# sikoba/babble

Measured on AMD Instinct MI355X. Metric: ECDSA event verifies/sec, higher is better.
Workload: dtype u32; 1 GPU; C2: VerifyBatch of 1M signed Events per GPU (64 creators, 1x64-B tx, ~446-B bodies); per-key tables rebuilt every step; events_per_gpu=1000000, creators=64, parallelism=single, batches_in_flight=2

## Files before the change

### babble_amd/csrc/bv_api.cpp

```cpp
#include "bv_internal.h"
#include "hostscalar.h"
#include "hostsha.h"

#include <algorithm>
#include <atomic>
#include <chrono>
#include <condition_variable>
#include <cstdio>
#include <cstdlib>
#include <cstring>
#include <functional>
#include <map>
#include <new>
#include <thread>

#include <sched.h>
#include <sys/syscall.h>
#include <unistd.h>

namespace {

constexpr uint64_t kGTableBytes = BV_GTABLE_U32 * 4;
constexpr uint64_t kGSubBytes = BV_GSUB_U32 * 4;
constexpr uint64_t kGPrefixBytes = (uint64_t)BV_GPAIR_BLOCKS * 4096 * 32;
constexpr uint64_t kKTableBytes = BV_KTABLE_U32 * 4;
constexpr uint64_t kK12TableBytes = BV_K12TABLE_U32 * 4;
constexpr uint64_t kK12SubBytes = BV_K12SUB_U32 * 4;
constexpr uint64_t kK12PrefixBytes = (uint64_t)BV_K12NWIN * BV_K12ENT * 32;
constexpr uint64_t kKSubBytes = BV_KSUB_U32 * 4;
constexpr uint64_t kKPrefixBytes = (uint64_t)BV_KNWIN * (1u << BV_KW) * 32;
constexpr uint32_t kBasesPerKey = 32;
constexpr uint32_t kMaxTableKeys = 8192;
constexpr uint32_t kMaxK12Keys = 1024;
constexpr uint32_t kManyKeys = 1024;
constexpr uint64_t kLatTableItems = 4096;
#ifndef BV_PREP_M
#define BV_PREP_M 16
#endif
constexpr uint32_t kPrepM = BV_PREP_M;
constexpr uint32_t kRgWords = 33;
#ifndef BV_FUSED_KC
#define BV_FUSED_KC 1
#endif
constexpr bool kFusedKc = BV_FUSED_KC;
constexpr size_t kChunk = 16ull << 20;
constexpr size_t kSmallStage = 1ull << 20;
constexpr uint64_t kHostHashLen = 16 << 10;

}

hipError_t DevBuf::ensure(size_t bytes) {
  if (bytes <= cap) return hipSuccess;
  if (p) {
    hipError_t e = hipFree(p);
    if (e != hipSuccess) return e;
    p = nullptr;
    cap = 0;
  }
  size_t want = std::max(bytes, cap * 3 / 2);
  want = (want + 255) & ~(size_t)255;
  hipError_t e = hipMalloc(&p, want);
  if (e != hipSuccess) {
    p = nullptr;
    (void)hipGetLastError();
    return e;
  }
  cap = want;
  return hipSuccess;
}
void DevBuf::release() {
  if (p) (void)hipFree(p);
  p = nullptr;
  cap = 0;
}
hipError_t PinnedBuf::ensure(size_t bytes) {
  if (bytes <= cap) return hipSuccess;
  if (p) {
    hipError_t e = hipHostFree(p);
    if (e != hipSuccess) return e;
    p = nullptr;
    cap = 0;
  }
  size_t want = std::max(bytes, cap * 3 / 2);
  want = (want + 4095) & ~(size_t)4095;
  hipError_t e = hipHostMalloc(&p, want, flags);
  if (e != hipSuccess) {
    p = nullptr;
    (void)hipGetLastError();
    return e;
  }
  cap = want;
  return hipSuccess;
}
void PinnedBuf::release() {
  if (p) (void)hipHostFree(p);
  p = nullptr;
  cap = 0;
}

int bv_fail(bv_ctx *c, int code, const char *what, hipError_t e) {
  if (c) {
    char buf[256];
    if (e != hipSuccess)
      snprintf(buf, sizeof buf, "%s: %s", what, hipGetErrorString(e));
    else
      snprintf(buf, sizeof buf, "%s", what);
    c->err = buf;
  }
  return code;
}

#define HIPCHK(expr, code, what)                               \
  do {                                                         \
    hipError_t _e = (expr);                                    \
    if (_e != hipSuccess) return bv_fail(ctx, code, what, _e); \
  } while (0)

namespace {
std::mutex g_pin_mu;
std::map<uintptr_t, size_t> g_pinned;
}

// ... 351 lines not shown
                    &sl.kc_tabs,   &sl.defer};
    for (auto *b : sb) b->release();
    sl.pin_small.release();
    if (sl.done) (void)hipEventDestroy(sl.done);
  }
  bv_kc_release(ctx);
  ctx->pin_in.release();
  ctx->pin_out.release();
  ctx->small_io.release();
  ctx->pin_long.release();
  ctx->d_long.release();
  for (auto &sl : ctx->slot)
    for (auto &e : sl.ev)
      if (e) (void)hipEventDestroy(e);
  for (auto &e : ctx->chunk_ev)
    if (e) (void)hipEventDestroy(e);
  if (ctx->ev_done) (void)hipEventDestroy(ctx->ev_done);
  if (ctx->ev_host) (void)hipEventDestroy(ctx->ev_host);
  streams_release(ctx);
  delete ctx->pool;
  delete ctx;
}

extern "C" void *bv_last_stream(const bv_ctx *ctx) { return ctx ? (void *)ctx->last : nullptr; }

static float elapsed(hipEvent_t a, hipEvent_t b);

extern "C" int bv_get_timing(const bv_ctx *ctx, bv_timing *out) {
  if (!ctx || !out) return BV_E_ARGS;
  bv_ctx *c = const_cast<bv_ctx *>(ctx);
  std::lock_guard<std::mutex> lk(c->mu);
  *out = c->timing;
  return BV_OK;
}

int bv_run_keys(bv_ctx *ctx, const bv_batch *b, hipEvent_t keys_ready, hipEvent_t s_ready, bool kc, bool split_ok) {
  const uint64_t n_items = b->n_items;
  const uint32_t n_keys = b->n_keys;
  if (n_items > 0 && (!b->item_msg || !b->item_key || !b->r_be || !b->s_be))
    return bv_fail(ctx, BV_E_ARGS, "null item arrays");
  if (n_items > 0 && n_keys == 0) return bv_fail(ctx, BV_E_ARGS, "items without keys");
  if (n_keys > 0 && !b->key_off) return bv_fail(ctx, BV_E_ARGS, "null key_off");
  if (((uintptr_t)b->r_be | (uintptr_t)b->s_be) & 15)
    return bv_fail(ctx, BV_E_ARGS, "r_be/s_be must be 16-byte aligned");
  HIPCHK(ctx->S().kstatus.ensure(std::max<uint32_t>(n_keys, 1)), BV_E_OOM, "alloc kstatus");
  HIPCHK(ctx->S().kxy.ensure(std::max<uint32_t>(n_keys, 1) * 64ull), BV_E_OOM, "alloc kxy");
  HIPCHK(ctx->S().scratch.ensure(std::max<uint64_t>(n_items, 1) * 32), BV_E_OOM, "alloc scratch");
  HIPCHK(ctx->S().u12.ensure(std::max<uint64_t>(n_items, 1) * BV_U_STRIDE * 4), BV_E_OOM, "alloc u12");

  const uint64_t min_items = n_keys <= kManyKeys ? ctx->table_min_items : ctx->table_min_items_many;
  const bool table_mode = kc || (n_keys <= kMaxTableKeys && n_items >= min_items * n_keys) ||
                          (n_keys <= ctx->lat_table_keys && n_items <= kLatTableItems && n_items > 0);
  const int key_w = kc ? BV_KCW
                    : !table_mode ? 0
                    : (n_keys <= kMaxK12Keys && n_items >= ctx->k12_min_items * n_keys && !(ctx->flags & BV_F_K8))
                        ? 12
                        : 8;
  ctx->table_mode = table_mode;
  ctx->key_w = key_w;
  if (table_mode) {
    HIPCHK(ctx->S().rg.ensure(std::max<uint64_t>(n_items, 1) * kRgWords * 4), BV_E_OOM, "alloc R_G");
    if (!kc) {
      const uint64_t nk = std::max<uint32_t>(n_keys, 1);
      HIPCHK(ctx->S().bases_jac.ensure(nk * kBasesPerKey * 96ull), BV_E_OOM, "alloc bases");
      HIPCHK(ctx->S().key_sub.ensure(nk * (key_w == 12 ? kK12SubBytes : kKSubBytes)), BV_E_OOM,
             "alloc key sub-tables");
      HIPCHK(ctx->S().key_pscr.ensure(nk * (key_w == 12 ? kK12PrefixBytes : kKPrefixBytes)), BV_E_OOM,
             "alloc key prefix scratch");
      HIPCHK(ctx->S().key_table.ensure(nk * (key_w == 12 ? kK12TableBytes : kKTableBytes)), BV_E_OOM,
             "alloc key tables");
    }
  }
  hipEvent_t *ev = ctx->S().ev;
  HIPCHK(hipStreamWaitEvent(ctx->sstream, keys_ready, 0), BV_E_LAUNCH, "fork");
  HIPCHK(hipEventRecord(ev[E_START], ctx->sstream), BV_E_LAUNCH, "event");
  if (kc && ctx->S().kc_decoded)
    HIPCHK(hipStreamWaitEvent(ctx->sstream, ctx->S().ev[E_KCDEC], 0), BV_E_LAUNCH, "join");
  else
    HIPCHK(bvk::key_decode(ctx->sstream, n_keys, b->key_bytes, b->key_off, ctx->S().kstatus.as<uint8_t>(),
                           ctx->S().kxy.as<uint32_t>()),
           BV_E_LAUNCH, "k_key_decode");
  HIPCHK(hipEventRecord(ev[E_KDEC], ctx->sstream), BV_E_LAUNCH, "event");
  HIPCHK(hipStreamWaitEvent(ctx->sstream, s_ready, 0), BV_E_LAUNCH, "fork");
  const uint32_t M = (uint32_t)std::min<uint64_t>(kPrepM, std::max<uint64_t>(1, (n_items + 65535) / 65536));
  HIPCHK(bvk::sinv(ctx->sstream, n_items, M, (const uint32_t *)b->s_be, b->pre, ctx->S().scratch.as<uint32_t>()),
         BV_E_LAUNCH, "k_sinv");
  ctx->S().glv_split = split_ok && ctx->glv_in_sstream && table_mode && !(kc && kFusedKc);
  if (ctx->S().glv_split)
    HIPCHK(bvk::glv_split(ctx->sstream, n_items, (const uint32_t *)b->r_be, ctx->S().scratch.as<uint32_t>(),
                          ctx->S().u12.as<uint32_t>()),
           BV_E_LAUNCH, "k_glv_split");
  HIPCHK(hipEventRecord(ev[E_SINV], ctx->sstream), BV_E_LAUNCH, "event");
  HIPCHK(hipStreamWaitEvent(ctx->kstream, ev[E_KDEC], 0), BV_E_LAUNCH, "fork");
  if (!kc) {
    if (table_mode)
      HIPCHK(bvk::build_tables(ctx->kstream, key_w, n_keys, ctx->S().kxy.as<uint32_t>(), ctx->S().kstatus.as<uint8_t>(),
                               ctx->S().bases_jac.as<uint32_t>(), ctx->S().key_sub.as<uint32_t>(),
                               ctx->S().key_pscr.as<uint32_t>(), ctx->S().key_table.as<uint32_t>(), n_items),
             BV_E_LAUNCH, "key tables");
  }
  HIPCHK(hipEventRecord(ev[E_KEYS], ctx->kstream), BV_E_LAUNCH, "event");
  return BV_OK;
}

int bv_out_bufs(bv_ctx *ctx, const bv_batch *b, uint8_t *d_msg_hash, uint8_t *d_status, uint64_t *d_bits,
                bool hashed, bv_out *o) {
  const uint64_t n_msgs = b->n_msgs, n_items = b->n_items;
  o->dig = (uint32_t *)d_msg_hash;
  if (hashed || !o->dig || ((uintptr_t)o->dig & 15)) {
    HIPCHK(ctx->S().digests.ensure(std::max<uint64_t>(n_msgs, 1) * 32), BV_E_OOM, "alloc digests");
    o->dig = ctx->S().digests.as<uint32_t>();
  }
  o->status = d_status;
  if (!o->status) {
    HIPCHK(ctx->S().status.ensure(std::max<uint64_t>(n_items, 1)), BV_E_OOM, "alloc status");
    o->status = ctx->S().status.as<uint8_t>();
  }
  o->bits = d_bits;
  if (!o->bits) {
    HIPCHK(ctx->S().bits.ensure(std::max<uint64_t>((n_items + 63) / 64, 1) * 8), BV_E_OOM, "alloc bits");
    o->bits = ctx->S().bits.as<uint64_t>();
  }
  return BV_OK;
}

int bv_launch_items(bv_ctx *ctx, const bv_batch *b, const bv_out &o, hipStream_t st, bool kc, uint64_t lo,
                    uint64_t hi, int part) {
  const uint64_t n = b->n_items;
  const uint8_t *kst = ctx->S().kstatus.as<uint8_t>();
  const uint32_t *r32 = (const uint32_t *)b->r_be, *s32 = (const uint32_t *)b->s_be;
  uint32_t *w = ctx->S().scratch.as<uint32_t>(), *u12 = ctx->S().u12.as<uint32_t>();
  const bool fused = kc && kFusedKc;
  if (part == 1) {
    if (ctx->table_mode && !fused)
      HIPCHK(bvk::verify_g(st, n, lo, hi, b->item_key, r32, s32, b->pre, kst, b->item_msg, o.dig, w, u12,
                           ctx->g_table, ctx->S().rg.as<uint32_t>(), ctx->S().glv_split),
             BV_E_LAUNCH, "k_verify_g");
    return BV_OK;
  }
  if (fused)
    HIPCHK(bvk::verify_gq(st, n, lo, hi, b->item_key, r32, s32, b->pre, kst, b->item_msg, o.dig, w, ctx->g_table,
                          ctx->S().kc_tabs.as<uint64_t>(), o.status, o.bits),
           BV_E_LAUNCH, "k_verify_gq");
  else if (ctx->table_mode)
    HIPCHK(bvk::verify_q(st, ctx->key_w, n, lo, hi, b->item_key, r32, s32, b->pre, kst, u12,
                         ctx->S().key_table.as<uint32_t>(), kc ? ctx->S().kc_tabs.as<uint64_t>() : nullptr,
                         ctx->S().rg.as<uint32_t>(), o.status, o.bits),
           BV_E_LAUNCH, "k_verify_q");
  else
    HIPCHK(bvk::verify_generic(st, n, lo, hi, b->item_key, r32, s32, b->pre, kst, ctx->S().kxy.as<uint32_t>(),
                               b->item_msg, o.dig, w, ctx->g_table, o.status, o.bits),
           BV_E_LAUNCH, "k_verify_generic");
  return BV_OK;
}

int bv_item_pipe::key_part(hipStream_t ks, hipEvent_t ready) {
  if (!ctx->table_mode || !ctx->qfirst || b->n_items == 0) return BV_OK;
  hipEvent_t *ev = ctx->S().ev;
  HIPCHK(hipStreamWaitEvent(ks, ev[E_SINV], 0), BV_E_LAUNCH, "join");
  HIPCHK(hipStreamWaitEvent(ks, ready, 0), BV_E_LAUNCH, "join");
  HIPCHK(hipStreamWaitEvent(ks, ev[E_KEYS], 0), BV_E_LAUNCH, "join");
  if (kc && ks != ctx->stream) {
    HIPCHK(hipEventRecord(ev[E_KCTAB], ctx->stream), BV_E_LAUNCH, "event");
    HIPCHK(hipStreamWaitEvent(ks, ev[E_KCTAB], 0), BV_E_LAUNCH, "join");
  }
  HIPCHK(hipEventRecord(ev[E_SCALAR], ks), BV_E_LAUNCH, "event");
  HIPCHK(hipEventRecord(ev[E_JOINED], ks), BV_E_LAUNCH, "event");
// ... 761 lines not shown
```

### babble_amd/csrc/field.h

```cpp
#pragma once
#include <hip/hip_runtime.h>
#include <stdint.h>

#define DEV __host__ __device__ __forceinline__

struct fe {
  uint32_t v[8];
};
struct sc {
  uint32_t v[8];
};
#if defined(__HIP_DEVICE_COMPILE__)
#include "field_asm.h"
#endif

#define P0 0xFFFFFC2Fu
#define P1 0xFFFFFFFEu
#define PX 0xFFFFFFFFu

DEV uint32_t addc32(uint32_t a, uint32_t b, uint32_t &c) {
  uint32_t co;
  uint32_t r = __builtin_addc(a, b, c, &co);
  c = co;
  return r;
// ... 312 lines not shown
#pragma unroll
    for (int j = 0; j < 8; j++) {
      uint64_t x = (uint64_t)a.v[i] * b.v[j] + t[j] + c;
      t[j] = (uint32_t)x;
      c = x >> 32;
    }
    uint32_t cc = 0;
    t[8] = addc32(t[8], (uint32_t)c, cc);
    t[9] = cc;
    uint32_t m = t[0] * SC_NINV;
    c = 0;
#pragma unroll
    for (int j = 0; j < 8; j++) {
      uint64_t x = (uint64_t)m * SC_N[j] + t[j] + c;
      t[j] = (uint32_t)x;
      c = x >> 32;
    }
    cc = 0;
    t[8] = addc32(t[8], (uint32_t)c, cc);
    t[9] += cc;
#pragma unroll
    for (int j = 0; j < 9; j++) t[j] = t[j + 1];
    t[9] = 0;
  }
#pragma unroll
  for (int i = 0; i < 8; i++) r.v[i] = t[i];
  if (t[8] || sc_ge_n(r)) sc_sub_n(r);
}

DEV void sc_load_const(sc &r, const uint32_t *c) {
#pragma unroll
  for (int i = 0; i < 8; i++) r.v[i] = c[i];
}

DEV void sc_add(sc &r, const sc &a, const sc &b) {
  uint32_t c = 0;
#pragma unroll
  for (int i = 0; i < 8; i++) r.v[i] = addc32(a.v[i], b.v[i], c);
  if (c || sc_ge_n(r)) sc_sub_n(r);
}
DEV void sc_sub(sc &r, const sc &a, const sc &b) {
  uint32_t br = 0;
#pragma unroll
  for (int i = 0; i < 8; i++) r.v[i] = subb32(a.v[i], b.v[i], br);
  if (br) {
    uint32_t c = 0;
#pragma unroll
    for (int i = 0; i < 8; i++) r.v[i] = addc32(r.v[i], SC_N[i], c);
  }
}

static constexpr uint32_t FE_BETA[8] = {0x719501EEu, 0xC1396C28u, 0x12F58995u, 0x9CF04975u,
                                        0xAC3434E9u, 0x6E64479Eu, 0x657C0710u, 0x7AE96A2Bu};
static constexpr uint32_t GLV_G1[8] = {0x45DBB031u, 0xE893209Au, 0x71E8CA7Fu, 0x3DAA8A14u,
                                       0x9284EB15u, 0xE86C90E4u, 0xA7D46BCDu, 0x3086D221u};
static constexpr uint32_t GLV_G2[8] = {0x8AC47F71u, 0x1571B4AEu, 0x9DF506C6u, 0x221208ACu,
                                       0x0ABFE4C4u, 0x6F547FA9u, 0x010E8828u, 0xE4437ED6u};
static constexpr uint32_t GLV_MB1R[8] = {0x0AD9263Cu, 0xC50468D0u, 0xFAA6ED42u, 0x1B1C8205u,
                                         0x8AC47F71u, 0x1571B4AEu, 0x9DF506C6u, 0x221208ACu};
static constexpr uint32_t GLV_MB2R[8] = {0x6A144696u, 0x0CAC5E50u, 0xF3BA5939u, 0x1E8A8DC5u,
                                         0xBA244FCEu, 0x176CDF65u, 0x8E173580u, 0xC25575EBu};
static constexpr uint32_t GLV_LAMR[8] = {0xC9926C9Eu, 0xF07DEB3Du, 0x83C6944Cu, 0x2C93E7ADu,
                                         0x52697D91u, 0x73A96606u, 0x8558D639u, 0x53284017u};
static constexpr uint32_t SC_HALF_N[8] = {0x681B20A0u, 0xDFE92F46u, 0x57A4501Du, 0x5D576E73u,
                                          0xFFFFFFFFu, 0xFFFFFFFFu, 0xFFFFFFFFu, 0x7FFFFFFFu};

DEV void glv_mulshift(sc &c, const sc &k, const uint32_t *g) {
  fe a, b;
  uint32_t w[16];
#pragma unroll
  for (int i = 0; i < 8; i++) {
    a.v[i] = k.v[i];
    b.v[i] = g[i];
  }
  mul_512(w, a, b);
  uint32_t cy = w[11] >> 31;
#pragma unroll
  for (int i = 0; i < 4; i++) c.v[i] = addc32(w[12 + i], 0u, cy);
  c.v[4] = cy;
#pragma unroll
  for (int i = 5; i < 8; i++) c.v[i] = 0;
}

DEV void glv_split(uint32_t mag1[4], uint32_t mag2[4], uint32_t &signs, const sc &k) {
  sc c1, c2, t, r1, r2, mb;
  glv_mulshift(c1, k, GLV_G1);
  glv_mulshift(c2, k, GLV_G2);
  sc_load_const(mb, GLV_MB1R);
  sc_mont(c1, c1, mb);
  sc_load_const(mb, GLV_MB2R);
  sc_mont(c2, c2, mb);
  sc_add(r2, c1, c2);
  sc_load_const(mb, GLV_LAMR);
  sc_mont(t, r2, mb);
  sc_sub(r1, k, t);
  signs = 0;
  sc h;
  sc_load_const(h, SC_HALF_N);
  sc n;
  sc_load_const(n, SC_N);
  bool gt1 = false, gt2 = false;
  {
    bool decided = false;
#pragma unroll
    for (int i = 7; i >= 0; i--) {
      if (!decided && r1.v[i] != h.v[i]) {
        gt1 = r1.v[i] > h.v[i];
        decided = true;
      }
    }
    decided = false;
#pragma unroll
    for (int i = 7; i >= 0; i--) {
      if (!decided && r2.v[i] != h.v[i]) {
        gt2 = r2.v[i] > h.v[i];
        decided = true;
      }
    }
  }
  if (gt1) {
    sc z;
    sc_sub(z, n, r1);
    r1 = z;
    signs |= 1u;
  }
  if (gt2) {
    sc z;
    sc_sub(z, n, r2);
    r2 = z;
    signs |= 2u;
  }
#pragma unroll
  for (int i = 0; i < 4; i++) {
    mag1[i] = r1.v[i];
    mag2[i] = r2.v[i];
  }
}

#include "modinv.h"

DEV void fe_inv_var(fe &r, const fe &a) {
  fe t = a;
  fe_canon(t);
  modinfo30 mi;
  modinfo_p(mi);
  modinv_var(r.v, t.v, mi);
}

static constexpr uint32_t SC_R3[8] = {0xE9FF41EDu, 0x7BC0CFE0u, 0x44D4322Cu, 0x00176484u,
                                      0xF1D0B2DAu, 0xB1B31347u, 0x18EF116Du, 0x555D800Cu};

DEV void sc_inverse_var(sc &r, const sc &xR) {
  modinfo30 mi;
  modinfo_n(mi);
  sc t, r3;
  modinv_var(t.v, xR.v, mi);
  sc_load_const(r3, SC_R3);
  sc_mont(r, t, r3);
}
```

### babble_amd/csrc/kernels.hip

```cpp
#include <hip/hip_runtime.h>
#include <stdint.h>

#include <algorithm>
#include <cstdlib>

#include "evjson.h"
#include "hostscalar.h"

#include "verify_core.h"


#ifndef BV_SHA_WAVES
#define BV_SHA_WAVES 1
#endif
__global__ void __launch_bounds__(256, BV_SHA_WAVES) k_sha256(uint64_t n_msgs, const uint8_t *__restrict__ bytes,
                                                const uint64_t *__restrict__ off,
                                                uint32_t *__restrict__ digest_words, uint64_t max_len) {
  const uint64_t m = (uint64_t)blockIdx.x * blockDim.x + threadIdx.x;
  if (m < n_msgs && off[m + 1] - off[m] <= max_len) sha256_one(m, bytes, off, digest_words);
}

__global__ void __launch_bounds__(256) k_put_digests(uint64_t n, const uint64_t *__restrict__ idx,
                                                     const uint32_t *__restrict__ vals, uint32_t *__restrict__ dig) {
  const uint64_t t = (uint64_t)blockIdx.x * blockDim.x + threadIdx.x;
// ... 160 lines not shown

template <bool LAT>
__global__ void __launch_bounds__(64) k_table_bases(uint32_t n_bases, const uint32_t *__restrict__ bxy,
                                                    const uint8_t *__restrict__ bstatus,
                                                    uint32_t *__restrict__ bases_jac, int w, int nwin) {
  const uint32_t b = blockIdx.x * blockDim.x + threadIdx.x;
  if (b >= n_bases) return;
  if (bstatus && bstatus[b] != KS_OK) return;
  table_bases_one<LAT>(b, bxy, bases_jac, w, nwin);
}

__global__ void __launch_bounds__(64) k_table_bases_coop(uint32_t n_bases, const uint32_t *__restrict__ bxy,
                                                         const uint8_t *__restrict__ bstatus,
                                                         uint32_t *__restrict__ bases_jac, int w, int nwin) {
  const uint32_t b = blockIdx.x;
  if (b >= n_bases) return;
  if (bstatus && bstatus[b] != KS_OK) return;
  coop_bases_one(b, bxy, bases_jac, w, nwin);
}

template <int N>
__device__ __forceinline__ void block_inverse(fe *T, fe &v, uint32_t t) {
  static_assert((N & (N - 1)) == 0, "power of two");
  T[N - 1 + t] = v;
  __syncthreads();
#pragma unroll 1
  for (uint32_t n = N / 2; n >= 1; n >>= 1) {
    if (t < n) {
      const uint32_t p = n - 1 + t;
      fe a = T[2 * p + 1], b = T[2 * p + 2], r;
      fe_mul(r, a, b);
      T[p] = r;
    }
    __syncthreads();
  }
  if (t == 0) {
    fe x, root = T[0];
    fe_inv_var(x, root);
    T[0] = x;
  }
  __syncthreads();
#pragma unroll 1
  for (uint32_t n = 1; n < N; n <<= 1) {
    const uint32_t c = 2 * n - 1 + t;
    fe r;
    if (t < 2 * n) {
      fe a = T[(c - 1) / 2], b = T[(c & 1u) ? c + 1 : c - 1];
      fe_mul(r, a, b);
    }
    __syncthreads();
    if (t < 2 * n) T[c] = r;
    __syncthreads();
  }
  v = T[N - 1 + t];
}

template <int W, int NWIN, bool PHI, int BLOCK = 256, bool LAT = true>
__global__ void __launch_bounds__(BLOCK) k_table_fill(const uint32_t *__restrict__ bases_jac,
                                                      const uint8_t *__restrict__ bstatus,
                                                      uint32_t *__restrict__ table) {
  static_assert(((NWIN << W) % BLOCK) == 0, "blocks cover whole keys");
  constexpr uint64_t half_u32 = (uint64_t)NWIN * (1ull << W) * BV_ENTRY_U32;
  const uint32_t b = blockIdx.y;
  const uint32_t f = blockIdx.x * BLOCK + threadIdx.x;
  const uint32_t j = f >> W;
  const uint32_t d = f & ((1u << W) - 1u);
  const uint32_t t = threadIdx.x;
  if (bstatus && bstatus[b] != KS_OK) return;
  __shared__ fe sT[2 * BLOCK - 1];
  const uint32_t *bj = bases_jac + ((uint64_t)b * NWIN + j) * 24;
  fe bx, by, bz;
  fe_load(bx, bj);
  fe_load(by, bj + 8);
  fe_load(bz, bj + 16);
  gej R;
  bool inf;
  fe Z;
  table_point<LAT>(R, inf, Z, bx, by, d, W);
  if (!inf) fe_mul(Z, Z, bz);
  fe zi = Z;
  block_inverse<BLOCK>(sT, zi, t);
  uint32_t *entry = table + (uint64_t)b * (PHI ? 2 : 1) * half_u32 + (((uint64_t)j << W) + d) * BV_ENTRY_U32;
  table_store(entry, PHI ? entry + half_u32 : nullptr, d, R, inf, zi);
}

template <int W, int L, int NWIN>
__global__ void __launch_bounds__(256) k_table_pair(const uint32_t *__restrict__ sub,
                                                    const uint8_t *__restrict__ bstatus,
                                                    uint32_t *__restrict__ table, uint4 *__restrict__ pscr) {
  constexpr uint32_t ENT = 1u << (W - 1), E = ENT / 256u, NS = 1u << L;
  constexpr uint64_t half_u32 = ((uint64_t)NWIN * ENT + 1) * BV_ENTRY_U32;
  static_assert(half_u32 == BV_K12HALF_U32, "K12 geometry");
  const uint32_t b = blockIdx.y, j = blockIdx.x, t = threadIdx.x;
  if (bstatus && bstatus[b] != KS_OK) return;
  const int live_bits = 128 - W * (int)j;
  const uint32_t e_live = live_bits >= W - 1 ? E : ((1u << live_bits) + 1u + 255u) / 256u;
  __shared__ uint32_t sLo[NS * BV_ENTRY_U32], sHi[NS * BV_ENTRY_U32];
  __shared__ fe sT[511];
  const uint32_t *sk = sub + ((uint64_t)b * 2 * NWIN + 2 * j) * NS * BV_ENTRY_U32;
  for (uint32_t x = t; x < NS * BV_ENTRY_U32; x += 256) {
    sLo[x] = sk[x];
    sHi[x] = sk[NS * BV_ENTRY_U32 + x];
  }
  __syncthreads();
  uint4 *ps = pscr + ((uint64_t)b * NWIN + j) * E * 2 * 256 + t;
  fe acc;
  fe_set(acc, 1);
#pragma unroll 1
  for (uint32_t e = 0; e < e_live; e++) {
    const uint32_t d = k12_digit(256 * e + t, ENT), lo = d & (NS - 1), hi = d >> L;
    fe x1, y1, x2, y2, H;
    pair_load(sLo, sHi, lo, hi, x1, y1, x2, y2);
    pair_denominator(H, pair_kind(lo, hi), x1, x2);
    ps[(2 * e) * 256] = make_uint4(acc.v[0], acc.v[1], acc.v[2], acc.v[3]);
    ps[(2 * e + 1) * 256] = make_uint4(acc.v[4], acc.v[5], acc.v[6], acc.v[7]);
    fe_mul(acc, acc, H);
  }
  fe q = acc;
  block_inverse<256>(sT, q, t);
  uint32_t *base = table + (uint64_t)b * 2 * half_u32 + (uint64_t)j * ENT * BV_ENTRY_U32;
#pragma unroll 1
  for (int e = (int)e_live - 1; e >= 0; e--) {
    const uint32_t d = k12_digit(256 * e + t, ENT), lo = d & (NS - 1), hi = d >> L;
    const int kind = pair_kind(lo, hi);
    fe x1, y1, x2, y2, H, Hinv, pre;
    pair_load(sLo, sHi, lo, hi, x1, y1, x2, y2);
    pair_denominator(H, kind, x1, x2);
    const uint4 p0 = ps[(2 * e) * 256], p1 = ps[(2 * e + 1) * 256];
    pre.v[0] = p0.x; pre.v[1] = p0.y; pre.v[2] = p0.z; pre.v[3] = p0.w;
    pre.v[4] = p1.x; pre.v[5] = p1.y; pre.v[6] = p1.z; pre.v[7] = p1.w;
    fe_mul(Hinv, q, pre);
    fe_mul(q, q, H);
    uint32_t *entry = base + (uint64_t)d * BV_ENTRY_U32;
    pair_store(entry, entry + half_u32, kind, x1, y1, x2, y2, Hinv);
  }
}

template <int W, int L, int NWIN, int WPB>
__global__ void __launch_bounds__(256) k_table_pair_u(const uint32_t *__restrict__ sub,
                                                      const uint8_t *__restrict__ bstatus,
                                                      uint32_t *__restrict__ table, uint4 *__restrict__ pscr) {
  constexpr uint32_t NS = 1u << L, SUB_U32 = 2 * WPB * NS * BV_ENTRY_U32;
  constexpr uint64_t half_u32 = (uint64_t)NWIN * (1ull << W) * BV_ENTRY_U32;
  static_assert((1u << W) == 256 && W == 2 * L && half_u32 == BV_KHALF_U32 && NWIN % WPB == 0, "K8 geometry");
  const uint32_t b = blockIdx.y, j0 = blockIdx.x * WPB, t = threadIdx.x;
  if (bstatus && bstatus[b] != KS_OK) return;
  __shared__ uint32_t sS[SUB_U32];
  __shared__ fe sT[511];
  const uint32_t *sk = sub + ((uint64_t)b * 2 * NWIN + 2 * j0) * NS * BV_ENTRY_U32;
  for (uint32_t x = t; x < SUB_U32; x += 256) sS[x] = sk[x];
  __syncthreads();
  const uint32_t lo = t & (NS - 1), hi = t >> L;
  const int kind = pair_kind(lo, hi);
  uint4 *ps = pscr + ((uint64_t)b * NWIN + j0) * 2 * 256 + t;
  fe acc;
  fe_set(acc, 1);
#pragma unroll 1
  for (uint32_t e = 0; e < WPB; e++) {
    fe x1, y1, x2, y2, H;
    pair_load(sS + 2 * e * NS * BV_ENTRY_U32, sS + (2 * e + 1) * NS * BV_ENTRY_U32, lo, hi, x1, y1, x2, y2);
    pair_denominator(H, kind, x1, x2);
    if (WPB > 1) {
      ps[(2 * e) * 256] = make_uint4(acc.v[0], acc.v[1], acc.v[2], acc.v[3]);
      ps[(2 * e + 1) * 256] = make_uint4(acc.v[4], acc.v[5], acc.v[6], acc.v[7]);
    }
    fe_mul(acc, acc, H);
// ... 825 lines not shown
  if (n == 0) return hipSuccess;
  hipLaunchKernelGGL(k_key_decode, grid1(n, 64), dim3(64), 0, st, n, kb, ko, kst, kxy);
  return hipGetLastError();
}

static int k12_lat_mask(bool busy) {
  static const int env = [] {
    const char *s = getenv("BV_K12_LAT");
    return s ? atoi(s) : -1;
  }();
  return env >= 0 ? env : busy ? 1 : 3;
}

static const bool g_coop_bases = [] {
  const char *s = getenv("BV_COOP_BASES");
  return s == nullptr || atoi(s) != 0;
}();

static const uint32_t g_k8_direct_keys = [] {
  const char *s = getenv("BV_K8_DIRECT_KEYS");
  return s ? (uint32_t)atoi(s) : 24u;
}();

hipError_t build_tables(hipStream_t st, int kw, uint32_t n_bases, const uint32_t *bxy, const uint8_t *bstatus,
                        uint32_t *bases_jac, uint32_t *sub, uint32_t *pscr, uint32_t *table, uint64_t n_items) {
  const bool k8_direct = kw == 8 && n_bases <= g_k8_direct_keys;
  if (n_bases == 0) return hipSuccess;
  const int w = kw == 0 ? BV_GL : kw == 8 ? (k8_direct ? BV_KW : BV_KL) : BV_K12L;
  const int nwin = kw == 0 ? BV_GNSUB : kw == 8 ? (k8_direct ? BV_KNWIN : BV_KNSUB) : BV_K12NSUB;
  const int lat = kw == 12 ? k12_lat_mask(!lat_variant(n_items)) : 3;
  if (g_coop_bases)
    hipLaunchKernelGGL(k_table_bases_coop, dim3(n_bases), dim3(64), 0, st, n_bases, bxy, bstatus, bases_jac, w, nwin);
  else if (lat & 1)
    hipLaunchKernelGGL(k_table_bases<true>, grid1(n_bases, 64), dim3(64), 0, st, n_bases, bxy, bstatus, bases_jac, w,
                       nwin);
  else
    hipLaunchKernelGGL(k_table_bases<false>, grid1(n_bases, 64), dim3(64), 0, st, n_bases, bxy, bstatus, bases_jac, w,
                       nwin);
  hipError_t e = hipGetLastError();
  if (e != hipSuccess) return e;
  if (kw == 0) {
    hipLaunchKernelGGL((k_table_fill<BV_GL, BV_GNSUB, false>), dim3(BV_GNSUB * ((1u << BV_GL) / 256u), 1), dim3(256),
                       0, st, bases_jac, bstatus, sub);
    e = hipGetLastError();
    if (e != hipSuccess) return e;
    for (uint32_t j = 0; j < BV_GNWIN; j++) {
      const int live_bits = 256 - BV_GW * (int)j;
      const uint64_t live = live_bits >= BV_GW - 1 ? BV_GENT : (1ull << live_bits) + 1;
      const uint32_t blocks = (uint32_t)((live + 4095) / 4096);
      for (uint32_t c0 = 0; c0 < blocks; c0 += BV_GPAIR_BLOCKS) {
        const uint32_t nb = blocks - c0 < BV_GPAIR_BLOCKS ? blocks - c0 : BV_GPAIR_BLOCKS;
        hipLaunchKernelGGL((k_table_pair_g<BV_GW, BV_GL>), dim3(nb), dim3(256), 0, st, sub, table, (uint4 *)pscr, j,
                           c0);
        e = hipGetLastError();
        if (e != hipSuccess) return e;
      }
    }
  } else if (k8_direct) {
    hipLaunchKernelGGL((k_table_fill<BV_KW, BV_KNWIN, true>), dim3(BV_KNWIN * ((1u << BV_KW) / 256u), n_bases),
                       dim3(256), 0, st, bases_jac, bstatus, table);
  } else if (kw == 8) {
    constexpr uint32_t fill_blocks = (BV_KNSUB << BV_KL) / 256u;
    if (lat_variant(n_items) && n_bases <= 256)
      hipLaunchKernelGGL((k_table_fill<BV_KL, BV_KNSUB, false, 256, true>), dim3(fill_blocks, n_bases), dim3(256), 0,
                         st, bases_jac, bstatus, sub);
    else
      hipLaunchKernelGGL((k_table_fill<BV_KL, BV_KNSUB, false, 256, false>), dim3(fill_blocks, n_bases), dim3(256), 0,
                         st, bases_jac, bstatus, sub);
    e = hipGetLastError();
    if (e != hipSuccess) return e;
    if (n_bases <= 64)
      hipLaunchKernelGGL((k_table_pair_u<BV_KW, BV_KL, BV_KNWIN, 1>), dim3(BV_KNWIN, n_bases), dim3(256), 0, st, sub,
                         bstatus, table, (uint4 *)pscr);
    else if (n_bases <= 256)
      hipLaunchKernelGGL((k_table_pair_u<BV_KW, BV_KL, BV_KNWIN, 4>), dim3(BV_KNWIN / 4, n_bases), dim3(256), 0, st, sub,
                         bstatus, table, (uint4 *)pscr);
    else
      hipLaunchKernelGGL((k_table_pair_u<BV_KW, BV_KL, BV_KNWIN, BV_KNWIN>), dim3(1, n_bases), dim3(256), 0, st, sub,
                         bstatus, table, (uint4 *)pscr);
  } else {
    if (lat & 2)
      hipLaunchKernelGGL((k_table_fill<BV_K12L, BV_K12NSUB, false, 1 << BV_K12L, true>), dim3(BV_K12NSUB, n_bases),
                         dim3(1 << BV_K12L), 0, st, bases_jac, bstatus, sub);
    else
      hipLaunchKernelGGL((k_table_fill<BV_K12L, BV_K12NSUB, false, 1 << BV_K12L, false>), dim3(BV_K12NSUB, n_bases),
                         dim3(1 << BV_K12L), 0, st, bases_jac, bstatus, sub);
    e = hipGetLastError();
    if (e != hipSuccess) return e;
    hipLaunchKernelGGL((k_table_pair<BV_K12W, BV_K12L, BV_K12NWIN>), dim3(BV_K12NWIN, n_bases), dim3(256), 0, st, sub,
                       bstatus, table, (uint4 *)pscr);
  }
  return hipGetLastError();
}

hipError_t sinv(hipStream_t st, uint64_t n, uint32_t M, const uint32_t *s_be, const uint8_t *pre, uint32_t *w) {
  if (n == 0) return hipSuccess;
  const uint64_t threads = (n + M - 1) / M;
  hipLaunchKernelGGL(k_sinv, grid1(threads, 256), dim3(256), 0, st, n, M, s_be, pre, w);
  return hipGetLastError();
}

hipError_t glv_split(hipStream_t st, uint64_t n, const uint32_t *r_be, const uint32_t *w, uint32_t *u12) {
  if (n == 0) return hipSuccess;
  hipLaunchKernelGGL(k_glv_split, grid1(n, 256), dim3(256), 0, st, n, r_be, w, u12);
  return hipGetLastError();
}

hipError_t verify_g(hipStream_t st, uint64_t n, uint64_t lo, uint64_t hi, const uint32_t *item_key,
                    const uint32_t *r_be, const uint32_t *s_be, const uint8_t *pre, const uint8_t *kst,
                    const uint32_t *item_msg, const uint32_t *dig, const uint32_t *w, uint32_t *u12,
                    const uint32_t *g_table, uint32_t *rg, bool split) {
  if (hi <= lo) return hipSuccess;
  const bool lat = lat_variant(n);
  auto k = lat ? (split ? k_verify_g<true, true> : k_verify_g<true, false>)
               : (split ? k_verify_g<false, true> : k_verify_g<false, false>);
  hipLaunchKernelGGL(k, grid1(hi - lo, 256), dim3(256), 0, st, n, lo, hi, item_key, r_be, s_be, pre, kst, item_msg,
                     dig, w, u12, g_table, rg);
  return hipGetLastError();
}

hipError_t verify_q(hipStream_t st, int kw, uint64_t n, uint64_t lo, uint64_t hi, const uint32_t *item_key,
                    const uint32_t *r_be, const uint32_t *s_be, const uint8_t *pre, const uint8_t *kst,
                    const uint32_t *u12, const uint32_t *key_table, const uint64_t *key_tabs, const uint32_t *rg,
                    uint8_t *status, uint64_t *bits) {
  if (hi <= lo) return hipSuccess;
  const bool lat = lat_variant(n);
#define BV_LAUNCH_Q(W, NWIN, KT, KTABS)                                                                             \
  if (lat)                                                                                                       \
    hipLaunchKernelGGL((k_verify_q<W, NWIN, true>), grid1(hi - lo, 256), dim3(256), 0, st, n, lo, hi, item_key,  \
                       r_be, s_be, pre, kst, u12, KT, KTABS, rg, status, bits);                                  \
  else                                                                                                           \
    hipLaunchKernelGGL((k_verify_q<W, NWIN, false>), grid1(hi - lo, 256), dim3(256), 0, st, n, lo, hi, item_key,   \
                       r_be, s_be, pre, kst, u12, KT, KTABS, rg, status, bits);
  if (kw == 8) {
    BV_LAUNCH_Q(BV_KW, BV_KNWIN, key_table, nullptr)
  } else if (kw == 12) {
    BV_LAUNCH_Q(BV_K12W, BV_K12NWIN, key_table, nullptr)
  } else {
    BV_LAUNCH_Q(BV_KCW, BV_KCNWIN, nullptr, key_tabs)
  }
#undef BV_LAUNCH_Q
  return hipGetLastError();
}

hipError_t verify_qf(hipStream_t st, int kw, uint64_t n, uint64_t lo, uint64_t hi, const uint32_t *item_key,
                     const uint32_t *r_be, const uint32_t *s_be, const uint8_t *pre, const uint8_t *kst,
                     const uint32_t *w, const uint32_t *key_table, const uint64_t *key_tabs, uint32_t *rq) {
  if (hi <= lo) return hipSuccess;
  const bool lat = lat_variant(n);
#define BV_LAUNCH_QF(W, NWIN, KT, KTABS)                                                                            \
  if (lat)                                                                                                       \
    hipLaunchKernelGGL((k_verify_qf<W, NWIN, true>), grid1(hi - lo, 256), dim3(256), 0, st, n, lo, hi, item_key, \
                       r_be, s_be, pre, kst, w, KT, KTABS, rq);                                                  \
  else                                                                                                           \
    hipLaunchKernelGGL((k_verify_qf<W, NWIN, false>), grid1(hi - lo, 256), dim3(256), 0, st, n, lo, hi, item_key, \
                       r_be, s_be, pre, kst, w, KT, KTABS, rq);
  if (kw == 8) {
    BV_LAUNCH_QF(BV_KW, BV_KNWIN, key_table, nullptr)
  } else if (kw == 12) {
    BV_LAUNCH_QF(BV_K12W, BV_K12NWIN, key_table, nullptr)
  } else {
    BV_LAUNCH_QF(BV_KCW, BV_KCNWIN, nullptr, key_tabs)
  }
#undef BV_LAUNCH_QF
  return hipGetLastError();
}

// ... 90 lines not shown
```

### babble_amd/csrc/verify_core.h

```cpp
#pragma once
#include <type_traits>
#include <stdint.h>

#include "../../include/babbleverify.h"
#include "geometry.h"
#include "coop.h"
#include "point.h"
#include "sha256.h"

#define KS_OK 0
#define KS_EMPTY 1
#define KS_BAD 2

static constexpr uint32_t P_MINUS_N[8] = {0x2FC9BAEEu, 0x402DA172u, 0x50B75FC4u, 0x45512319u,
                                          0x00000001u, 0u, 0u, 0u};

DEV void fe_load_be(fe &r, const uint8_t *b) {
#pragma unroll
  for (int i = 0; i < 8; i++) {
    const uint8_t *q = b + 4 * (7 - i);
    r.v[i] = ((uint32_t)q[0] << 24) | ((uint32_t)q[1] << 16) | ((uint32_t)q[2] << 8) | q[3];
  }
}
DEV void fe_load_be_words(fe &r, const uint32_t *w) {
// ... 152 lines not shown
  fe zi2, zi3, x, y;
  fe_sqr(zi2, zi);
  fe_mul(zi3, zi2, zi);
  fe_mul(x, R.X, zi2);
  fe_mul(y, R.Y, zi3);
  fe_canon(x);
  fe_canon(y);
  if (d == 0 || inf) {
    fe_set(x, 0);
    fe_set(y, 0);
  }
  uint32_t v[16];
#pragma unroll
  for (int i = 0; i < 8; i++) {
    v[i] = x.v[i];
    v[8 + i] = y.v[i];
  }
  store16(entry, v);
  if (phi) {
    fe beta, bx;
    fe_load(beta, FE_BETA);
    fe_mul(bx, x, beta);
    fe_canon(bx);
#pragma unroll
    for (int i = 0; i < 8; i++) v[i] = bx.v[i];
    store16(phi, v);
  }
}

DEV int pair_kind(uint32_t lo, uint32_t hi) { return (lo ? 1 : 0) | (hi ? 2 : 0); }

DEV uint32_t k12_digit(uint32_t d, uint32_t ent) { return d ? d : ent; }

DEV void pair_load(const uint32_t *s_lo, const uint32_t *s_hi, uint32_t lo, uint32_t hi, fe &x1, fe &y1, fe &x2,
                   fe &y2) {
  fe_load(x1, s_lo + BV_ENTRY_U32 * lo);
  fe_load(y1, s_lo + BV_ENTRY_U32 * lo + 8);
  fe_load(x2, s_hi + BV_ENTRY_U32 * hi);
  fe_load(y2, s_hi + BV_ENTRY_U32 * hi + 8);
}

DEV void pair_denominator(fe &H, int kind, const fe &x1, const fe &x2) {
  if (kind == 3) fe_sub(H, x2, x1);
  else fe_set(H, 1);
}

DEV void pair_store(uint32_t *entry, uint32_t *phi, int kind, const fe &x1, const fe &y1, const fe &x2, const fe &y2,
                    const fe &Hinv) {
  fe x, y;
  if (kind == 3) {
    fe lam, t;
    fe_sub(t, y2, y1);
    fe_mul(lam, t, Hinv);
    fe_sqr(x, lam);
    fe_sub(x, x, x1);
    fe_sub(x, x, x2);
    fe_sub(t, x1, x);
    fe_mul(y, lam, t);
    fe_sub(y, y, y1);
  } else if (kind == 1) {
    x = x1;
    y = y1;
  } else {
    x = x2;
    y = y2;
  }
  fe_canon(x);
  fe_canon(y);
  uint32_t v[16];
#pragma unroll
  for (int i = 0; i < 8; i++) {
    v[i] = x.v[i];
    v[8 + i] = y.v[i];
  }
  store16(entry, v);
  if (!phi) return;
  fe beta, bx;
  fe_load(beta, FE_BETA);
  fe_mul(bx, x, beta);
  fe_canon(bx);
#pragma unroll
  for (int i = 0; i < 8; i++) v[i] = bx.v[i];
  store16(phi, v);
}

DEV void sc_sqrn(sc &a, int n) {
#pragma unroll 1
  for (int i = 0; i < n; i++) sc_mont(a, a, a);
}

DEV void sc_inverse(sc &r, const sc &x) {
  sc x2, x3, x5, x7, x9, x11, x13, x15;
  sc_mont(x2, x, x);
  sc_mont(x3, x2, x);
  sc_mont(x5, x3, x2);
  sc_mont(x7, x5, x2);
  sc_mont(x9, x7, x2);
  sc_mont(x11, x9, x2);
  sc_mont(x13, x11, x2);
  sc_mont(x15, x13, x2);
  sc a2 = x3, a4, a8, a16, a32, a64, t;
  a4 = a2; sc_sqrn(a4, 2); sc_mont(a4, a4, a2);
  a8 = a4; sc_sqrn(a8, 4); sc_mont(a8, a8, a4);
  a16 = a8; sc_sqrn(a16, 8); sc_mont(a16, a16, a8);
  a32 = a16; sc_sqrn(a32, 16); sc_mont(a32, a32, a16);
  a64 = a32; sc_sqrn(a64, 32); sc_mont(a64, a64, a32);
  t = a64;
  sc_sqrn(t, 32); sc_mont(t, t, a32);
  sc_sqrn(t, 16); sc_mont(t, t, a16);
  sc_sqrn(t, 8); sc_mont(t, t, a8);
  sc_sqrn(t, 4); sc_mont(t, t, a4);
  sc_sqrn(t, 2); sc_mont(t, t, a2);
  sc_sqrn(t, 1); sc_mont(t, t, x);
  sc_sqrn(t, 1);
#define SQM(n, m) sc_sqrn(t, n); sc_mont(t, t, m);
  SQM(4, x11) SQM(3, x5) SQM(4, x5) SQM(4, x7) SQM(5, x13) SQM(2, x3) SQM(5, x7) SQM(6, x13)
  SQM(5, x11) SQM(4, x13) SQM(3, x) SQM(6, x5) SQM(10, x7) SQM(4, x7) SQM(5, x15) SQM(4, x15)
  SQM(5, x9) SQM(6, x11) SQM(4, x13) SQM(5, x3) SQM(6, x13) SQM(10, x13) SQM(4, x9) SQM(9, x9)
  SQM(4, x15) SQM(1, x)
#undef SQM
  r = t;
}

DEV bool s_usable(const uint8_t *pre, uint64_t i, const sc &s) {
  return (pre == nullptr || pre[i] == 0) && !u256_is_zero(s.v) && u256_lt(s.v, SC_N);
}

DEV void sinv_thread(uint64_t t, uint64_t T, uint64_t n_items, uint32_t M, const uint32_t *s_be, const uint8_t *pre,
                     uint32_t *w_out) {
  sc R1, one;
  sc_load_const(R1, SC_R1);
#pragma unroll
  for (int k = 0; k < 8; k++) one.v[k] = k == 0 ? 1u : 0u;
  sc acc = R1;
  for (uint32_t m = 0; m < M; m++) {
    const uint64_t i = t + (uint64_t)m * T;
    if (i >= n_items) break;
    sc s;
    sc_load_be_words(s, s_be + 8 * i);
    if (!s_usable(pre, i, s)) s = one;
    uint4 *q = (uint4 *)(w_out + 8 * i);
    q[0] = make_uint4(acc.v[0], acc.v[1], acc.v[2], acc.v[3]);
    q[1] = make_uint4(acc.v[4], acc.v[5], acc.v[6], acc.v[7]);
    sc_mont(acc, acc, s);
  }
  sc inv;
  sc_inverse_var(inv, acc);
  sc_mont(inv, inv, one);
  for (int m = (int)M - 1; m >= 0; m--) {
    const uint64_t i = t + (uint64_t)m * T;
    if (i >= n_items) continue;
    sc s, pfx, w;
    sc_load_be_words(s, s_be + 8 * i);
    if (!s_usable(pre, i, s)) s = one;
    uint4 *q = (uint4 *)(w_out + 8 * i);
    const uint4 a = q[0], b = q[1];
    pfx.v[0] = a.x; pfx.v[1] = a.y; pfx.v[2] = a.z; pfx.v[3] = a.w;
    pfx.v[4] = b.x; pfx.v[5] = b.y; pfx.v[6] = b.z; pfx.v[7] = b.w;
    sc_mont(w, inv, pfx);
    sc_mont(inv, inv, s);
    q[0] = make_uint4(w.v[0], w.v[1], w.v[2], w.v[3]);
    q[1] = make_uint4(w.v[4], w.v[5], w.v[6], w.v[7]);
  }
}

DEV void item_scalars(uint64_t i, const uint32_t *r_be, const uint32_t *item_msg, const uint32_t *digest_words,
// ... 666 lines not shown
```

Baseline: 531.9 million verifies/s.

## Use integer GLV split and shared-multiple K12 table fill

```diff
diff --git a/babble_amd/csrc/bv_api.cpp b/babble_amd/csrc/bv_api.cpp
--- a/babble_amd/csrc/bv_api.cpp
+++ b/babble_amd/csrc/bv_api.cpp
@@ -38,6 +38,10 @@
 #define BV_PREP_M 16
 #endif
 constexpr uint32_t kPrepM = BV_PREP_M;
+#ifndef BV_PREP_LANES
+#define BV_PREP_LANES 65536
+#endif
+constexpr uint64_t kPrepLanes = BV_PREP_LANES;
 constexpr uint32_t kRgWords = 33;
 #ifndef BV_FUSED_KC
 #define BV_FUSED_KC 1
@@ -555,7 +559,8 @@
            BV_E_LAUNCH, "k_key_decode");
   HIPCHK(hipEventRecord(ev[E_KDEC], ctx->sstream), BV_E_LAUNCH, "event");
   HIPCHK(hipStreamWaitEvent(ctx->sstream, s_ready, 0), BV_E_LAUNCH, "fork");
-  const uint32_t M = (uint32_t)std::min<uint64_t>(kPrepM, std::max<uint64_t>(1, (n_items + 65535) / 65536));
+  const uint32_t M =
+      (uint32_t)std::min<uint64_t>(kPrepM, std::max<uint64_t>(1, (n_items + kPrepLanes - 1) / kPrepLanes));
   HIPCHK(bvk::sinv(ctx->sstream, n_items, M, (const uint32_t *)b->s_be, b->pre, ctx->S().scratch.as<uint32_t>()),
          BV_E_LAUNCH, "k_sinv");
   ctx->S().glv_split = split_ok && ctx->glv_in_sstream && table_mode && !(kc && kFusedKc);
diff --git a/babble_amd/csrc/field.h b/babble_amd/csrc/field.h
--- a/babble_amd/csrc/field.h
+++ b/babble_amd/csrc/field.h
@@ -418,7 +418,7 @@
   for (int i = 5; i < 8; i++) c.v[i] = 0;
 }
 
-DEV void glv_split(uint32_t mag1[4], uint32_t mag2[4], uint32_t &signs, const sc &k) {
+DEV void glv_split_mont(uint32_t mag1[4], uint32_t mag2[4], uint32_t &signs, const sc &k) {
   sc c1, c2, t, r1, r2, mb;
   glv_mulshift(c1, k, GLV_G1);
   glv_mulshift(c2, k, GLV_G2);
@@ -473,6 +473,59 @@
   }
 }
 
+#ifndef BV_GLV_INT
+#define BV_GLV_INT 1
+#endif
+static constexpr uint32_t GLV_NB1[5] = {0x0ABFE4C3u, 0x6F547FA9u, 0x010E8828u, 0xE4437ED6u, 0x00000000u};
+static constexpr uint32_t GLV_NA1[5] = {0x6D7B14EBu, 0x17936F1Bu, 0x582B9432u, 0xCF792DDEu, 0xFFFFFFFFu};
+static constexpr uint32_t GLV_NA2[5] = {0x62BB3028u, 0xA83EEF72u, 0x571D0C09u, 0xEB35AF08u, 0xFFFFFFFEu};
+
+DEV void glv_macc5(uint32_t w[5], const uint32_t a[5], const uint32_t b[5]) {
+#pragma unroll
+  for (int i = 0; i < 5; i++) {
+    uint64_t c = 0;
+#pragma unroll
+    for (int j = 0; i + j < 5; j++) {
+      uint64_t t = (uint64_t)a[i] * b[j] + w[i + j] + c;
+      w[i + j] = (uint32_t)t;
+      c = t >> 32;
+    }
+  }
+}
+
+DEV bool glv_abs5(uint32_t mag[4], const uint32_t w[5]) {
+  const uint32_t m = 0u - (w[4] >> 31);
+  uint32_t c = m & 1u;
+#pragma unroll
+  for (int i = 0; i < 4; i++) mag[i] = addc32(w[i] ^ m, 0u, c);
+  return m != 0;
+}
+
+DEV void glv_split_int(uint32_t mag1[4], uint32_t mag2[4], uint32_t &signs, const sc &k) {
+  sc c1, c2;
+  glv_mulshift(c1, k, GLV_G1);
+  glv_mulshift(c2, k, GLV_G2);
+  uint32_t w1[5], w2[5];
+#pragma unroll
+  for (int i = 0; i < 5; i++) {
+    w1[i] = k.v[i];
+    w2[i] = 0;
+  }
+  glv_macc5(w1, c1.v, GLV_NA1);
+  glv_macc5(w1, c2.v, GLV_NA2);
+  glv_macc5(w2, c1.v, GLV_NB1);
+  glv_macc5(w2, c2.v, GLV_NA1);
+  signs = (glv_abs5(mag1, w1) ? 1u : 0u) | (glv_abs5(mag2, w2) ? 2u : 0u);
+}
+
+DEV void glv_split(uint32_t mag1[4], uint32_t mag2[4], uint32_t &signs, const sc &k) {
+#if BV_GLV_INT
+  glv_split_int(mag1, mag2, signs, k);
+#else
+  glv_split_mont(mag1, mag2, signs, k);
+#endif
+}
+
 #include "modinv.h"
 
 DEV void fe_inv_var(fe &r, const fe &a) {
diff --git a/babble_amd/csrc/kernels.hip b/babble_amd/csrc/kernels.hip
--- a/babble_amd/csrc/kernels.hip
+++ b/babble_amd/csrc/kernels.hip
@@ -266,6 +266,46 @@
   block_inverse<BLOCK>(sT, zi, t);
   uint32_t *entry = table + (uint64_t)b * (PHI ? 2 : 1) * half_u32 + (((uint64_t)j << W) + d) * BV_ENTRY_U32;
   table_store(entry, PHI ? entry + half_u32 : nullptr, d, R, inf, zi);
+}
+
+template <int NSUB>
+__global__ void __launch_bounds__(64) k_fill_multiples(const uint32_t *__restrict__ bases_jac,
+                                                       const uint8_t *__restrict__ bstatus,
+                                                       uint32_t *__restrict__ mult) {
+  const uint32_t b = blockIdx.y, u = blockIdx.x * 64 + threadIdx.x;
+  if (bstatus && bstatus[b] != KS_OK) return;
+  if (u < (uint32_t)BV_FS_MULTS * NSUB) fill_multiple_one<NSUB>(b, u, bases_jac, mult);
+}
+
+template <int W, int L, int NSUB>
+__global__ void __launch_bounds__(64) k_table_fill_shared(const uint32_t *__restrict__ bases_jac,
+                                                          const uint8_t *__restrict__ bstatus,
+                                                          const uint32_t *__restrict__ mult,
+                                                          uint32_t *__restrict__ table) {
+  static_assert(L == 6, "the multiples are 3 + 3 bits");
+  constexpr uint32_t ODD = BV_FS_ODD_LIVE(W, L), LIVE = fs_live<L, NSUB, ODD>();
+  constexpr uint64_t key_u32 = (uint64_t)NSUB * (1ull << L) * BV_ENTRY_U32;
+  const uint32_t b = blockIdx.y, t = threadIdx.x, f = blockIdx.x * 64 + t;
+  if (bstatus && bstatus[b] != KS_OK) return;
+  __shared__ fe sT[2 * 64 - 1];
+  const bool live = f < LIVE;
+  uint32_t k = 0, x = 0;
+  if (live) fill_shared_slot<L, NSUB, ODD>(f, k, x);
+  gej R;
+  bool inf = true;
+  fe Z;
+  fe_set(Z, 1);
+  if (live) {
+    fill_shared_point<NSUB>(R, inf, Z, b, k, x, mult);
+    if (!inf) {
+      fe bz;
+      fe_load(bz, bases_jac + ((uint64_t)b * NSUB + k) * 24 + 16);
+      fe_mul(Z, Z, bz);
+    }
+  }
+  fe zi = Z;
+  block_inverse<64>(sT, zi, t);
+  if (live) table_store(table + (uint64_t)b * key_u32 + (((uint64_t)k << L) + x) * BV_ENTRY_U32, nullptr, x, R, inf, zi);
 }
 
 template <int W, int L, int NWIN>
@@ -1257,7 +1297,17 @@
     if (lat & 2)
       hipLaunchKernelGGL((k_table_fill<BV_K12L, BV_K12NSUB, false, 1 << BV_K12L, true>), dim3(BV_K12NSUB, n_bases),
                          dim3(1 << BV_K12L), 0, st, bases_jac, bstatus, sub);
-    else
+    else if (BV_FILL_SHARED) {
+      constexpr uint32_t live = fs_live<BV_K12L, BV_K12NSUB, BV_FS_ODD_LIVE(BV_K12W, BV_K12L)>();
+      static_assert(BV_K12L == 6 && fs_mult_u32<BV_K12NSUB>() * 4 <= (uint64_t)BV_K12NWIN * BV_K12ENT * 32,
+                    "multiples fit the K12 prefix scratch");
+      hipLaunchKernelGGL((k_fill_multiples<BV_K12NSUB>), dim3((BV_FS_MULTS * BV_K12NSUB + 63) / 64, n_bases), dim3(64), 0,
+                         st, bases_jac, bstatus, pscr);
+      e = hipGetLastError();
+      if (e != hipSuccess) return e;
+      hipLaunchKernelGGL((k_table_fill_shared<BV_K12W, BV_K12L, BV_K12NSUB>), dim3((live + 63) / 64, n_bases), dim3(64),
+                         0, st, bases_jac, bstatus, pscr, sub);
+    } else
       hipLaunchKernelGGL((k_table_fill<BV_K12L, BV_K12NSUB, false, 1 << BV_K12L, false>), dim3(BV_K12NSUB, n_bases),
                          dim3(1 << BV_K12L), 0, st, bases_jac, bstatus, sub);
     e = hipGetLastError();
diff --git a/babble_amd/csrc/verify_core.h b/babble_amd/csrc/verify_core.h
--- a/babble_amd/csrc/verify_core.h
+++ b/babble_amd/csrc/verify_core.h
@@ -258,6 +258,77 @@
 #pragma unroll
   for (int i = 0; i < 8; i++) v[i] = bx.v[i];
   store16(phi, v);
+}
+
+#ifndef BV_FILL_SHARED
+#define BV_FILL_SHARED 1
+#endif
+#define BV_FS_MULTS 14
+#define BV_FS_ODD_LIVE(W, L) ((1u << ((W) - (L) - 1)) + 1u)
+
+template <int NSUB>
+DEV constexpr uint64_t fs_mult_u32() { return (uint64_t)NSUB * BV_FS_MULTS * 24; }
+template <int L, int NSUB, uint32_t ODD>
+DEV constexpr uint32_t fs_live() { return (uint32_t)((NSUB + 1) / 2) * (1u << L) + (uint32_t)(NSUB / 2) * ODD; }
+
+template <int NSUB>
+DEV void fill_multiple_one(uint32_t b, uint32_t u, const uint32_t *bases_jac, uint32_t *mult) {
+  const bool big = u >= 7u * NSUB;
+  const uint32_t v = big ? u - 7u * NSUB : u, k = v / 7u, i = v % 7u;
+  const uint32_t *bj = bases_jac + ((uint64_t)b * NSUB + k) * 24;
+  fe bx, by, Z;
+  fe_load(bx, bj);
+  fe_load(by, bj + 8);
+  gej R;
+  bool inf;
+  table_point<false>(R, inf, Z, bx, by, big ? 8u * (i + 1) : i + 1, 6);
+  uint32_t *o = mult + (uint64_t)b * fs_mult_u32<NSUB>() + ((uint64_t)k * BV_FS_MULTS + (big ? 7u : 0u) + i) * 24;
+  fe_store(o, R.X);
+  fe_store(o + 8, R.Y);
+  fe_store(o + 16, Z);
+}
+
+template <int L, int NSUB, uint32_t ODD>
+DEV void fill_shared_slot(uint32_t f, uint32_t &k, uint32_t &x) {
+  constexpr uint32_t EVEN = (uint32_t)((NSUB + 1) / 2) << L;
+  if (f < EVEN) {
+    k = 2u * (f >> L);
+    x = f & ((1u << L) - 1u);
+  } else {
+    k = 2u * ((f - EVEN) / ODD) + 1u;
+    x = (f - EVEN) % ODD;
+  }
+}
+
+template <int NSUB>
+DEV void fill_shared_point(gej &R, bool &inf, fe &Z, uint32_t b, uint32_t k, uint32_t x, const uint32_t *mult) {
+  const uint32_t l = x & 7u, h = x >> 3;
+  const uint32_t *mk = mult + (uint64_t)b * fs_mult_u32<NSUB>() + (uint64_t)k * BV_FS_MULTS * 24;
+  inf = x == 0;
+  fe_set(R.X, 0);
+  fe_set(R.Y, 0);
+  fe_set(R.Z, 1);
+  if (l) {
+    const uint32_t *p = mk + (l - 1u) * 24;
+    fe_load(R.X, p);
+    fe_load(R.Y, p + 8);
+    fe_load(R.Z, p + 16);
+  }
+  if (h) {
+    const uint32_t *p = mk + (7u + h - 1u) * 24;
+    gej H;
+    fe_load(H.X, p);
+    fe_load(H.Y, p + 8);
+    fe_load(H.Z, p + 16);
+    if (l) {
+      bool ri = false;
+      gej_add(R, ri, H, false);
+      inf = ri;
+    } else {
+      R = H;
+    }
+  }
+  Z = R.Z;
 }
 
 DEV void sc_sqrn(sc &a, int n) {
```

After: 540.6 million verifies/s, median of 6. +1.6%, better.
